# zxhuang1698/ShapeClipper

Measured on AMD Instinct MI355X. Metric: train-step images/sec (Pix3D cfg, bs32/GPU), higher is better.
Workload: dtype f32 (bf16x3-split MFMA, fp32 accumulate)

## Files before the change

### shapeclipper_amd/csrc/conv3x3_wgrad.hip

```cpp
#include <hip/hip_runtime.h>

#include "grid_cus.hpp"
#include "shapeclipper_hip.h"

namespace sc {

typedef float wg_f32x16 __attribute__((ext_vector_type(16)));

#ifdef SC_WGRAD_PROFILE
__device__ unsigned long long* wgrad_prof_buf = nullptr;
#define WG_STAMP(ID) { const unsigned long long t_ = __builtin_amdgcn_s_memrealtime(); if (wgrad_prof_buf && tid == 0) wgrad_prof_buf[(size_t)blockIdx.x * 16 + (ID)] = t_; }
#define WG_ACCUM(ID, T0) { const unsigned long long t_ = __builtin_amdgcn_s_memrealtime(); if (wgrad_prof_buf && tid == 0) wgrad_prof_buf[(size_t)blockIdx.x * 16 + (ID)] += t_ - (T0); }
#else
#define WG_STAMP(ID)
#endif

template <int W_, int NR_, int NIMG_, int GS_, int S_ = 1>
struct WgCfg {
    static constexpr int W = W_, H = W_, NR = NR_, NIMG = NIMG_, GS = GS_, S = S_;
    static constexpr int HW = W * W;
    static constexpr int XW = S * W, XH = S * H, XHW = XW * XH;
    static constexpr int Wp = S == 1 ? W + 2 : XW + 1;
    static constexpr bool WHOLE = NR == H;
    static constexpr int SLOTW = (W + 2 * GS - 1) / (2 * GS) * (2 * GS);
    static constexpr int ROWS = NIMG * NR;
    static constexpr int NSLOT = ROWS * SLOTW;
    static constexpr int GST = NSLOT + (((NSLOT / GS) & 1) ? 0 : GS);
    static constexpr int PR = S == 1 ? NR + 2 : 2 * NR + 1;
    static constexpr int PATCH = NIMG * PR * Wp;
    static constexpr int LQ = (S == 1 ? PATCH : PATCH + 2 * GS + 2) | 1;
    static constexpr int LDS_FLOATS = 64 * GST + 64 * LQ > 4 * 48 * 64 ? 64 * GST + 64 * LQ : 4 * 48 * 64;
    static constexpr int CHUNK = W == 7 ? 49 : 56;
    static constexpr int RPC = CHUNK / W;
    static constexpr int XCHUNK = XW == 7 ? 49 : 56, XRPC = XCHUNK / XW;
    static constexpr int XROWS = WHOLE ? XH : PR;
    static constexpr int XCH = (XROWS + XRPC - 1) / XRPC, GCH = (NR + RPC - 1) / RPC;
    static constexpr int HR = ROWS / 2;
    static constexpr int GPR = SLOTW / (2 * GS);
    static constexpr int KH_A = HR * SLOTW;
    static constexpr int KH_B = NIMG == 2 ? PR * Wp : S * HR * Wp;
    static constexpr int NBV = S == 1 ? GS + 2 : 2 * GS + 1;
    static_assert(ROWS % 2 == 0 && H % NR == 0 && SLOTW % (2 * GS) == 0 && CHUNK % W == 0 && XCHUNK % XW == 0 && (S == 1 || S == 2), "K-step shape");
    static_assert(LDS_FLOATS * 4 <= 160 * 1024 && 4 * 48 * 64 <= LDS_FLOATS, "LDS");
};

template <class C>
__global__ __launch_bounds__(512, 1) void conv3x3_wgrad_kernel(const float* __restrict__ gy, const float* __restrict__ x,
                                                               float* __restrict__ partial, int batch, int cin, int cout, int S) {
    constexpr int W = C::W, H = C::H, HW = C::HW, Wp = C::Wp, GS = C::GS, NIMG = C::NIMG, NR = C::NR, ST = C::S;
    constexpr int XW = C::XW, XH = C::XH, XHW = C::XHW;
    extern __shared__ float4 wg_smem[];
    float* As = reinterpret_cast<float*>(wg_smem);
    float* Xs = As + 64 * C::GST;
    const int tid = threadIdx.x, lane = tid & 63, wave = __builtin_amdgcn_readfirstlane(tid >> 6), half = lane >> 5;
    const int wt = wave & 3, kh = wave >> 2;
    const int nti = cin / 64;
    const int blk = blockIdx.x / S, s = blockIdx.x - blk * S;
    const int co0 = (blk / nti) * 64, ci0 = (blk % nti) * 64;
    const int nimg_steps = NIMG == 2 ? (batch + 1) / 2 : batch * (H / NR);
    const int k_lo = (int)((long long)s * nimg_steps / S), k_hi = (int)((long long)(s + 1) * nimg_steps / S);

    for (int i = tid; i < C::LDS_FLOATS; i += 512) As[i] = 0.f;

    const bool lane_on = lane < C::CHUNK, xlane_on = lane < C::XCHUNK;
    const int lrow = lane / W, lx = lane - lrow * W;
    const int xlrow = lane / XW, xlx = lane - xlrow * XW;
    float xv[8][C::XCH * NIMG], gv[8][C::GCH * NIMG];
    auto load = [&](int kstep) {
        int b, y0;
        if (NIMG == 2) { b = 2 * kstep; y0 = 0; } else { b = kstep / (H / NR); y0 = (kstep - b * (H / NR)) * NR; }
#pragma unroll
        for (int im = 0; im < NIMG; ++im) {
            const bool img_ok = b + im < batch;
            const float* xb = x + ((size_t)(b + im) * cin + ci0 + 8 * wave) * XHW;
            const float* gb = gy + ((size_t)(b + im) * cout + co0 + 8 * wave) * HW;
#pragma unroll
            for (int c = 0; c < C::XCH; ++c) {
                const int yr = (C::WHOLE ? 0 : ST * y0 - 1) + c * C::XRPC + xlrow;
                const bool ok = xlane_on && img_ok && (unsigned)yr < (unsigned)XH && c * C::XRPC + xlrow < C::XROWS;
                const int off = yr * XW + xlx;
#pragma unroll
                for (int ch = 0; ch < 8; ++ch) xv[ch][im * C::XCH + c] = ok ? xb[ch * XHW + off] : 0.f;
            }
#pragma unroll
            for (int c = 0; c < C::GCH; ++c) {
                const int yr = y0 + c * C::RPC + lrow;
                const bool ok = lane_on && img_ok && c * C::RPC + lrow < NR;
                const int off = yr * W + lx;
#pragma unroll
                for (int ch = 0; ch < 8; ++ch) gv[ch][im * C::GCH + c] = ok ? gb[ch * HW + off] : 0.f;
            }
        }
    };
    auto store = [&]() {
#pragma unroll
        for (int im = 0; im < NIMG; ++im) {
#pragma unroll
            for (int c = 0; c < C::XCH; ++c) {
                const int pr = (C::WHOLE ? 1 : 0) + c * C::XRPC + xlrow;
                if (xlane_on && c * C::XRPC + xlrow < C::XROWS) {
#pragma unroll
                    for (int ch = 0; ch < 8; ++ch) Xs[(8 * wave + ch) * C::LQ + (im * C::PR + pr) * Wp + 1 + xlx] = xv[ch][im * C::XCH + c];
                }
            }
#pragma unroll
            for (int c = 0; c < C::GCH; ++c) {
                if (lane_on && c * C::RPC + lrow < NR) {
#pragma unroll
                    for (int ch = 0; ch < 8; ++ch) As[(8 * wave + ch) * C::GST + (im * NR + c * C::RPC + lrow) * C::SLOTW + lx] = gv[ch][im * C::GCH + c];
                }
            }
        }
    };

    wg_f32x16 acc[9];
#pragma unroll
    for (int t = 0; t < 9; ++t)
#pragma unroll
        for (int r = 0; r < 16; ++r) acc[t][r] = 0.f;

    const float* Ab = As + ((wt >> 1) * 32 + (lane & 31)) * C::GST + half * GS + kh * C::KH_A;
    const float* Bb = Xs + ((wt & 1) * 32 + (lane & 31)) * C::LQ + half * ST * GS + kh * C::KH_B;

    if (k_lo < k_hi) load(k_lo);
    __syncthreads();
    for (int kstep = k_lo; kstep < k_hi; ++kstep) {
        store();
        __syncthreads();
        if (kstep + 1 < k_hi) load(kstep + 1);
#pragma unroll
        for (int yr = 0; yr < C::HR; ++yr) {
#pragma unroll
            for (int gx = 0; gx < C::GPR; ++gx) {
                float a[GS];
                if constexpr (GS == 4) {
                    const float4 t = *reinterpret_cast<const float4*>(Ab + yr * C::SLOTW + gx * 8);
                    a[0] = t.x, a[1] = t.y, a[2] = t.z, a[3] = t.w;
                } else if constexpr (GS == 2) {
                    const float2 t = *reinterpret_cast<const float2*>(Ab + yr * C::SLOTW + gx * 4);
                    a[0] = t.x, a[1] = t.y;
                } else {
                    a[0] = Ab[yr * C::SLOTW + gx * 2];
                }
#pragma unroll
                for (int ky = 0; ky < 3; ++ky) {
                    float bv[C::NBV];
#pragma unroll
                    for (int t = 0; t < C::NBV; ++t) bv[t] = Bb[(ST * yr + ky) * Wp + ST * gx * 2 * GS + t];
#pragma unroll
                    for (int ss = 0; ss < GS; ++ss)
#pragma unroll
                        for (int kx = 0; kx < 3; ++kx)
                            acc[ky * 3 + kx] = __builtin_amdgcn_mfma_f32_32x32x2f32(a[ss], bv[ST * ss + kx], acc[ky * 3 + kx], 0, 0, 0);
                }
            }
        }
        __syncthreads();
    }

    float* R = As;
#pragma unroll
    for (int pass = 0; pass < 3; ++pass) {
        if (kh == 1) {
#pragma unroll
            for (int t = 0; t < 3; ++t)
#pragma unroll
                for (int r = 0; r < 16; ++r) R[((wt * 3 + t) * 16 + r) * 64 + lane] = acc[pass * 3 + t][r];
        }
        __syncthreads();
        if (kh == 0) {
#pragma unroll
            for (int t = 0; t < 3; ++t)
#pragma unroll
                for (int r = 0; r < 16; ++r) acc[pass * 3 + t][r] += R[((wt * 3 + t) * 16 + r) * 64 + lane];
        }
        __syncthreads();
    }
    if (kh == 0) {
        float* dst = partial + (size_t)blockIdx.x * (64 * 64 * 9);
#pragma unroll
        for (int t = 0; t < 9; ++t)
#pragma unroll
            for (int r = 0; r < 16; ++r) dst[((wt * 9 + t) * 16 + r) * 64 + lane] = acc[t][r];
    }
}

__global__ __launch_bounds__(256) void conv3x3_wgrad_reduce_kernel(const float* __restrict__ partial, float* __restrict__ dw, int cin,
                                                                  int cout, int S) {
    __shared__ float part[4][64];
    const int nti = cin / 64, lane = threadIdx.x & 63, w = threadIdx.x >> 6;
    const int blk = blockIdx.x / 576, e = (blockIdx.x - blk * 576) * 64 + lane;
    const float* src = partial + (size_t)blk * S * 36864 + e;
    float s0 = 0.f, s1 = 0.f;
    int s = w;
    for (; s + 4 < S; s += 8) {
        s0 += src[(size_t)s * 36864];
        s1 += src[(size_t)(s + 4) * 36864];
    }
    if (s < S) s0 += src[(size_t)s * 36864];
    part[w][lane] = s0 + s1;
    __syncthreads();
    if (w == 0) {
        const float sum = (part[0][lane] + part[1][lane]) + (part[2][lane] + part[3][lane]);
        const int r = (e >> 6) & 15, t = (e >> 10) % 9, wt = e / (9 * 1024);
        const int co = (blk / nti) * 64 + (wt >> 1) * 32 + (r & 3) + 8 * (r >> 2) + 4 * (lane >> 5);
        const int ci = (blk % nti) * 64 + (wt & 1) * 32 + (lane & 31);
        dw[((size_t)co * cin + ci) * 9 + t] = sum;
    }
}

using Wg56 = WgCfg<56, 2, 1, 4>;
using Wg28 = WgCfg<28, 4, 1, 2>;
using Wg14 = WgCfg<14, 14, 1, 1>;
using Wg7 = WgCfg<7, 7, 2, 1>;
using Wg28S2 = WgCfg<28, 2, 1, 2, 2>;
using Wg14S2 = WgCfg<14, 2, 1, 1, 2>;
using Wg7S2 = WgCfg<7, 7, 2, 1, 2>;

typedef __bf16 wg_bf16x8 __attribute__((ext_vector_type(8)));
typedef float wg_f32x4 __attribute__((ext_vector_type(4)));
#ifndef SC_WGRAD_S16
#define SC_WGRAD_S16 0
#endif

template <int W_, int NR_, int NIMG_>
struct WsCfg {
    static constexpr int W = W_, H = W_, NR = NR_, NIMG = NIMG_, HW = W * W;
    static constexpr int SLOTS = W == 7 ? 8 : (W + 15) / 16 * 16;
    static constexpr int ROWS = NIMG * NR, NSLOT = ROWS * SLOTS, G = NSLOT / 16;
    static constexpr int ASTR = NSLOT + 8;
    static constexpr int Wp = SLOTS + 2, PR = NR + 2, PATCH = NIMG * PR * Wp;
    static constexpr int BSTR = (PATCH + 3) / 4 * 4 + 2;
    static constexpr bool WHOLE = NR == H;
    static constexpr int LDS_BYTES = 3 * 64 * (ASTR + BSTR) * 2;
    static constexpr int CHUNK = W == 7 ? 49 : 56, RPC = CHUNK / W;
    static constexpr int XROWS = WHOLE ? H : PR;
    static constexpr int XCH = (XROWS + RPC - 1) / RPC, GCH = (NR + RPC - 1) / RPC;
    static_assert(NSLOT % 16 == 0 && H % NR == 0 && LDS_BYTES <= 160 * 1024 && (W >= 14 || (NIMG == 2 && NR == 7)), "K-step shape");
    static constexpr int boff(int g, int h) {
        if (W == 7) { const int r = 2 * g + h; return ((r / 7) * PR + r % 7) * Wp; }
        const int r = g / (SLOTS / 16), gx = g % (SLOTS / 16);
        return ((r / NR) * PR + r % NR) * Wp + 16 * gx + 8 * h;
    }
};

template <class C>
__global__ __launch_bounds__(768, 1) void conv3x3_wgrad_split_kernel(const float* __restrict__ gy, const float* __restrict__ x,
                                                                     float* __restrict__ partial, int batch, int cin, int cout, int S) {
    constexpr int W = C::W, H = C::H, HW = C::HW, Wp = C::Wp, NIMG = C::NIMG, NR = C::NR;
    extern __shared__ float4 wg_smem[];
    __bf16* As = reinterpret_cast<__bf16*>(wg_smem);
    __bf16* Xs = As + 3 * 64 * C::ASTR;
    const int tid = threadIdx.x, lane = tid & 63, wave = __builtin_amdgcn_readfirstlane(tid >> 6), half = lane >> 5;
    const int wt = wave & 3, ky = wave >> 2;
    const int nti = cin / 64;
    const int blk = blockIdx.x / S, s = blockIdx.x - blk * S;
    const int co0 = (blk / nti) * 64, ci0 = (blk % nti) * 64;
    const int nimg_steps = NIMG == 2 ? (batch + 1) / 2 : batch * (H / NR);
    const int k_lo = (int)((long long)s * nimg_steps / S), k_hi = (int)((long long)(s + 1) * nimg_steps / S);

    for (int i = tid; i < C::LDS_BYTES / 16; i += 768) wg_smem[i] = make_float4(0.f, 0.f, 0.f, 0.f);

    const bool lane_on = lane < C::CHUNK, xrole = wave < 8;
    const int lrow = lane / W, lx = lane - lrow * W;
    constexpr int NSV = 8 * C::XCH * NIMG > 16 * C::GCH * NIMG ? 8 * C::XCH * NIMG : 16 * C::GCH * NIMG;
    float sv[NSV];
    auto load = [&](int kstep) {
        int b, y0;
        if (NIMG == 2) { b = 2 * kstep; y0 = 0; } else { b = kstep / (H / NR); y0 = (kstep - b * (H / NR)) * NR; }
        if (xrole) {
#pragma unroll
            for (int im = 0; im < NIMG; ++im) {
                const float* xb = x + ((size_t)(b + im) * cin + ci0 + 8 * wave) * HW;
#pragma unroll
                for (int c = 0; c < C::XCH; ++c) {
                    const int rr = c * C::RPC + lrow, yr = (C::WHOLE ? 0 : y0 - 1) + rr;
                    const bool ok = lane_on && b + im < batch && (unsigned)yr < (unsigned)H && rr < C::XROWS;
                    const int off = yr * W + lx;
#pragma unroll
                    for (int ch = 0; ch < 8; ++ch) sv[(im * C::XCH + c) * 8 + ch] = ok ? xb[ch * HW + off] : 0.f;
                }
            }
        } else {
#pragma unroll
            for (int im = 0; im < NIMG; ++im) {
                const float* gb = gy + ((size_t)(b + im) * cout + co0 + 16 * (wave - 8)) * HW;
#pragma unroll
                for (int c = 0; c < C::GCH; ++c) {
                    const int rr = c * C::RPC + lrow;
                    const bool ok = lane_on && b + im < batch && rr < NR;
                    const int off = (y0 + rr) * W + lx;
#pragma unroll
                    for (int ch = 0; ch < 16; ++ch) sv[(im * C::GCH + c) * 16 + ch] = ok ? gb[ch * HW + off] : 0.f;
                }
            }
        }
    };
    auto put = [&](__bf16* d, int stride, float v) {
        const __bf16 h0 = (__bf16)v;
        const float r1 = v - (float)h0;
        const __bf16 h1 = (__bf16)r1;
        d[0] = h0; d[stride] = h1; d[2 * stride] = (__bf16)(r1 - (float)h1);
    };
    auto store = [&]() {
        if (xrole) {
#pragma unroll
            for (int im = 0; im < NIMG; ++im)
#pragma unroll
                for (int c = 0; c < C::XCH; ++c) {
                    const int rr = c * C::RPC + lrow;
                    if (lane_on && rr < C::XROWS) {
                        __bf16* d = Xs + 8 * wave * C::BSTR + (im * C::PR + (C::WHOLE ? 1 : 0) + rr) * Wp + 1 + lx;
#pragma unroll
                        for (int ch = 0; ch < 8; ++ch) put(d + ch * C::BSTR, 64 * C::BSTR, sv[(im * C::XCH + c) * 8 + ch]);
                    }
                }
        } else {
#pragma unroll
            for (int im = 0; im < NIMG; ++im)
#pragma unroll
                for (int c = 0; c < C::GCH; ++c) {
                    const int rr = c * C::RPC + lrow;
                    if (lane_on && rr < NR) {
                        __bf16* d = As + 16 * (wave - 8) * C::ASTR + (im * NR + rr) * C::SLOTS + lx;
#pragma unroll
                        for (int ch = 0; ch < 16; ++ch) put(d + ch * C::ASTR, 64 * C::ASTR, sv[(im * C::GCH + c) * 16 + ch]);
                    }
                }
        }
    };

#if SC_WGRAD_S16
    wg_f32x4 acc[3][2][2];
#pragma unroll
    for (int t = 0; t < 3; ++t)
#pragma unroll
        for (int u = 0; u < 4; ++u) acc[t][u >> 1][u & 1] = wg_f32x4{0.f, 0.f, 0.f, 0.f};
    const int q4 = lane >> 4, l16 = lane & 15;
    const __bf16* Ab = As + ((wt >> 1) * 32 + l16) * C::ASTR + 8 * q4;
    const unsigned* Bb = reinterpret_cast<const unsigned*>(Xs + ((wt & 1) * 32 + l16) * C::BSTR + ky * Wp);
#else
    wg_f32x16 acc[3];
#pragma unroll
    for (int t = 0; t < 3; ++t)
#pragma unroll
        for (int r = 0; r < 16; ++r) acc[t][r] = 0.f;

    const __bf16* Ab = As + ((wt >> 1) * 32 + (lane & 31)) * C::ASTR + 8 * half;
    const unsigned* Bb = reinterpret_cast<const unsigned*>(Xs + ((wt & 1) * 32 + (lane & 31)) * C::BSTR + ky * Wp);
#endif

    WG_STAMP(0)
    if (k_lo < k_hi) load(k_lo);
    __syncthreads();
    WG_STAMP(1)
    for (int kstep = k_lo; kstep < k_hi; ++kstep) {
#ifdef SC_WGRAD_PROFILE
        const unsigned long long ts0 = __builtin_amdgcn_s_memrealtime();
#endif
        store();
        __syncthreads();
#ifdef SC_WGRAD_PROFILE
        WG_ACCUM(4, ts0)
        const unsigned long long ts1 = __builtin_amdgcn_s_memrealtime();
#endif
        if (kstep + 1 < k_hi) load(kstep + 1);
#if SC_WGRAD_S16
#pragma unroll
        for (int G2 = 0; G2 < (C::G + 1) / 2; ++G2) {
            constexpr int NG = C::G;
            const bool tail = 2 * G2 + 1 >= NG;
            const bool dead = tail && q4 >= 2;
            const int g1 = tail ? 2 * G2 : 2 * G2 + 1;
            const int bo = (q4 == 0 ? C::boff(2 * G2, 0) : q4 == 1 ? C::boff(2 * G2, 1) : q4 == 2 ? C::boff(g1, 0) : C::boff(g1, 1)) >> 1;
            float4 a[3][2];
#pragma unroll
            for (int pc = 0; pc < 3; ++pc)
#pragma unroll
                for (int u = 0; u < 2; ++u) {
                    const float4 av = *reinterpret_cast<const float4*>(Ab + pc * 64 * C::ASTR + u * 16 * C::ASTR + (dead ? 0 : 32 * G2));
                    a[pc][u] = dead ? make_float4(0.f, 0.f, 0.f, 0.f) : av;
                }
#pragma unroll
            for (int sb = 0; sb < 2; ++sb) {
                unsigned d[3][5];
#pragma unroll
                for (int pc = 0; pc < 3; ++pc)
#pragma unroll
                    for (int q = 0; q < 5; ++q) d[pc][q] = Bb[pc * 32 * C::BSTR + sb * 8 * C::BSTR + bo + q];
#pragma unroll
                for (int term = 0; term < 6; ++term) {
                    constexpr int PA[6] = {0, 2, 1, 0, 1, 0}, PB[6] = {2, 0, 1, 1, 0, 0};
                    const unsigned* q = d[PB[term]];
                    const uint4 b0 = {q[0], q[1], q[2], q[3]}, b2 = {q[1], q[2], q[3], q[4]};
                    const uint4 b1 = {__builtin_amdgcn_alignbit(q[1], q[0], 16), __builtin_amdgcn_alignbit(q[2], q[1], 16),
                                      __builtin_amdgcn_alignbit(q[3], q[2], 16), __builtin_amdgcn_alignbit(q[4], q[3], 16)};
#pragma unroll
                    for (int sa = 0; sa < 2; ++sa) {
                        const wg_bf16x8 av = __builtin_bit_cast(wg_bf16x8, a[PA[term]][sa]);
                        acc[0][sa][sb] = __builtin_amdgcn_mfma_f32_16x16x32_bf16(av, __builtin_bit_cast(wg_bf16x8, b0), acc[0][sa][sb], 0, 0, 0);
                        acc[1][sa][sb] = __builtin_amdgcn_mfma_f32_16x16x32_bf16(av, __builtin_bit_cast(wg_bf16x8, b1), acc[1][sa][sb], 0, 0, 0);
                        acc[2][sa][sb] = __builtin_amdgcn_mfma_f32_16x16x32_bf16(av, __builtin_bit_cast(wg_bf16x8, b2), acc[2][sa][sb], 0, 0, 0);
                    }
                }
#pragma unroll
                for (int pc = 0; pc < 3; ++pc)
                    asm volatile("" : "+v"(acc[0][0][sb]) : "v"(d[pc][0]), "v"(d[pc][1]), "v"(d[pc][2]), "v"(d[pc][3]), "v"(d[pc][4]));
            }
#pragma unroll
            for (int pc = 0; pc < 3; ++pc)
                asm volatile("" : "+v"(acc[0][0][0]) : "v"(__builtin_bit_cast(wg_f32x4, a[pc][0])), "v"(__builtin_bit_cast(wg_f32x4, a[pc][1])));
            __builtin_amdgcn_sched_barrier(0);
        }
#else
#pragma unroll
        for (int g = 0; g < C::G; ++g) {
            float4 a[3];
            unsigned d[3][5];
            const int bo = (half ? C::boff(g, 1) : C::boff(g, 0)) >> 1;
#pragma unroll
            for (int pc = 0; pc < 3; ++pc) {
                a[pc] = *reinterpret_cast<const float4*>(Ab + pc * 64 * C::ASTR + 16 * g);
#pragma unroll
                for (int q = 0; q < 5; ++q) d[pc][q] = Bb[pc * 32 * C::BSTR + bo + q];
            }
#pragma unroll
            for (int term = 0; term < 6; ++term) {
                constexpr int PA[6] = {0, 2, 1, 0, 1, 0}, PB[6] = {2, 0, 1, 1, 0, 0};
                const unsigned* q = d[PB[term]];
                const wg_bf16x8 av = __builtin_bit_cast(wg_bf16x8, a[PA[term]]);
                uint4 b0 = {q[0], q[1], q[2], q[3]}, b2 = {q[1], q[2], q[3], q[4]};
                uint4 b1 = {__builtin_amdgcn_alignbit(q[1], q[0], 16), __builtin_amdgcn_alignbit(q[2], q[1], 16),
                            __builtin_amdgcn_alignbit(q[3], q[2], 16), __builtin_amdgcn_alignbit(q[4], q[3], 16)};
                acc[0] = __builtin_amdgcn_mfma_f32_32x32x16_bf16(av, __builtin_bit_cast(wg_bf16x8, b0), acc[0], 0, 0, 0);
                acc[1] = __builtin_amdgcn_mfma_f32_32x32x16_bf16(av, __builtin_bit_cast(wg_bf16x8, b1), acc[1], 0, 0, 0);
                acc[2] = __builtin_amdgcn_mfma_f32_32x32x16_bf16(av, __builtin_bit_cast(wg_bf16x8, b2), acc[2], 0, 0, 0);
            }
        }
#endif
        __syncthreads();
#ifdef SC_WGRAD_PROFILE
        WG_ACCUM(5, ts1)
#endif
    }
    WG_STAMP(2)
    float* dst = partial + (size_t)blockIdx.x * (64 * 64 * 9);
#if SC_WGRAD_S16
#pragma unroll
    for (int t = 0; t < 3; ++t)
#pragma unroll
        for (int sa = 0; sa < 2; ++sa)
#pragma unroll
            for (int sb = 0; sb < 2; ++sb)
#pragma unroll
                for (int r = 0; r < 4; ++r)
                    dst[((wt * 9 + ky * 3 + t) * 16 + r + 4 * (2 * sa + (q4 >> 1))) * 64 + 16 * sb + l16 + 32 * (q4 & 1)] = acc[t][sa][sb][r];
#else
#pragma unroll
    for (int t = 0; t < 3; ++t)
#pragma unroll
        for (int r = 0; r < 16; ++r) dst[((wt * 9 + ky * 3 + t) * 16 + r) * 64 + lane] = acc[t][r];
#endif
#ifdef SC_WGRAD_PROFILE
    asm volatile("s_waitcnt vmcnt(0)" ::: "memory");
    WG_STAMP(3)
    if (wgrad_prof_buf && tid == 0) wgrad_prof_buf[(size_t)blockIdx.x * 16 + 6] = (unsigned long long)(k_hi - k_lo);
#endif
}

using Ws56 = WsCfg<56, 2, 1>;
using Ws28 = WsCfg<28, 4, 1>;
using Ws14 = WsCfg<14, 7, 1>;
using Ws7 = WsCfg<7, 7, 2>;

static int wg_cus() { return grid_cus(); }
static int wg_splits(int cin, int cout) {
    const int nblk = (cin / 64) * (cout / 64), s = wg_cus() / nblk;
    return s > 0 ? s : 1;
}

template <class C>
static int launch_wgrad(const float* gy, const float* x, float* dw, float* workspace, int batch, int cin, int cout, hipStream_t st) {
    if (cin % 64 || cout % 64 || batch <= 0) return (int)hipErrorInvalidValue;
    const int nblk = (cin / 64) * (cout / 64), S = wg_splits(cin, cout);
    (void)hipFuncSetAttribute((const void*)conv3x3_wgrad_kernel<C>, hipFuncAttributeMaxDynamicSharedMemorySize, C::LDS_FLOATS * 4);
    hipLaunchKernelGGL((conv3x3_wgrad_kernel<C>), dim3(nblk * S), dim3(512), C::LDS_FLOATS * 4, st, gy, x, workspace, batch, cin, cout, S);
    hipLaunchKernelGGL(conv3x3_wgrad_reduce_kernel, dim3(nblk * 576), dim3(256), 0, st, workspace, dw, cin, cout, S);
    return (int)hipGetLastError();
}

template <class C>
static int launch_wgrad_split(const float* gy, const float* x, float* dw, float* workspace, int batch, int cin, int cout, hipStream_t st) {
    if (cin % 64 || cout % 64 || batch <= 0) return (int)hipErrorInvalidValue;
    const int nblk = (cin / 64) * (cout / 64), S = wg_splits(cin, cout);
    (void)hipFuncSetAttribute((const void*)conv3x3_wgrad_split_kernel<C>, hipFuncAttributeMaxDynamicSharedMemorySize, C::LDS_BYTES);
    hipLaunchKernelGGL((conv3x3_wgrad_split_kernel<C>), dim3(nblk * S), dim3(768), C::LDS_BYTES, st, gy, x, workspace, batch, cin, cout, S);
    hipLaunchKernelGGL(conv3x3_wgrad_reduce_kernel, dim3(nblk * 576), dim3(256), 0, st, workspace, dw, cin, cout, S);
    return (int)hipGetLastError();
}

}

#ifdef SC_WGRAD_PROFILE
extern "C" int sc_wgrad_debug_set_prof(unsigned long long* buf) {
    return (int)hipMemcpyToSymbol(HIP_SYMBOL(sc::wgrad_prof_buf), &buf, sizeof(buf));
}
#endif
extern "C" int sc_conv3x3_wgrad_split(const float* gy, const float* x, float* dw, float* workspace, int batch, int cin, int cout, int hw, void* stream) {
    switch (hw) {
        case 56: return sc::launch_wgrad_split<sc::Ws56>(gy, x, dw, workspace, batch, cin, cout, (hipStream_t)stream);
        case 28: return sc::launch_wgrad_split<sc::Ws28>(gy, x, dw, workspace, batch, cin, cout, (hipStream_t)stream);
        case 14: return sc::launch_wgrad_split<sc::Ws14>(gy, x, dw, workspace, batch, cin, cout, (hipStream_t)stream);
        case 7: return sc::launch_wgrad_split<sc::Ws7>(gy, x, dw, workspace, batch, cin, cout, (hipStream_t)stream);
        default: return -1;
    }
}

extern "C" long long sc_conv3x3_wgrad_workspace_floats(int cin, int cout) {
    if (cin <= 0 || cout <= 0 || cin % 64 || cout % 64) return -1;
    return (long long)(cin / 64) * (cout / 64) * sc::wg_splits(cin, cout) * 36864;
}

extern "C" int sc_conv3x3s2_wgrad(const float* gy, const float* x, float* dw, float* workspace, int batch, int cin, int cout, int hw, void* stream) {
    switch (hw) {
        case 56: return sc::launch_wgrad<sc::Wg28S2>(gy, x, dw, workspace, batch, cin, cout, (hipStream_t)stream);
        case 28: return sc::launch_wgrad<sc::Wg14S2>(gy, x, dw, workspace, batch, cin, cout, (hipStream_t)stream);
        case 14: return sc::launch_wgrad<sc::Wg7S2>(gy, x, dw, workspace, batch, cin, cout, (hipStream_t)stream);
        default: return -1;
    }
}

extern "C" int sc_conv3x3_wgrad(const float* gy, const float* x, float* dw, float* workspace, int batch, int cin, int cout, int hw, void* stream) {
    switch (hw) {
        case 56: return sc::launch_wgrad<sc::Wg56>(gy, x, dw, workspace, batch, cin, cout, (hipStream_t)stream);
        case 28: return sc::launch_wgrad<sc::Wg28>(gy, x, dw, workspace, batch, cin, cout, (hipStream_t)stream);
        case 14: return sc::launch_wgrad<sc::Wg14>(gy, x, dw, workspace, batch, cin, cout, (hipStream_t)stream);
        case 7: return sc::launch_wgrad<sc::Wg7>(gy, x, dw, workspace, batch, cin, cout, (hipStream_t)stream);
        default: return -1;
    }
}
```

Baseline: 1037.

## Deal wgrad staging loads across waves in channel pairs and precompute B-operand addresses

Adds a paired load and store path for the split wgrad kernel, used by the 28 and 14 configs. Each wave now loads contiguous pixel runs for pairs of channels, with both wave classes sharing the x and gy work, and splits two values at once into bf16x3 using packed converts and 32-bit LDS stores. It also removes the unused 16x16 MFMA variant and reworks the B-operand fetch to two 4-word loads from precomputed byte offsets, deriving the shifted operand by alignbit. This is meant to cut global-load imbalance, per-element split cost and LDS address arithmetic, at the price of more template parameters and higher register pressure in the staging buffer.

```diff
diff --git a/shapeclipper_amd/csrc/conv3x3_wgrad.hip b/shapeclipper_amd/csrc/conv3x3_wgrad.hip
--- a/shapeclipper_amd/csrc/conv3x3_wgrad.hip
+++ b/shapeclipper_amd/csrc/conv3x3_wgrad.hip
@@ -218,12 +218,10 @@
 using Wg7S2 = WgCfg<7, 7, 2, 1, 2>;
 
 typedef __bf16 wg_bf16x8 __attribute__((ext_vector_type(8)));
-typedef float wg_f32x4 __attribute__((ext_vector_type(4)));
-#ifndef SC_WGRAD_S16
-#define SC_WGRAD_S16 0
-#endif
-
-template <int W_, int NR_, int NIMG_>
+typedef __bf16 wg_bf16x2 __attribute__((ext_vector_type(2)));
+typedef float wg_f32x2 __attribute__((ext_vector_type(2)));
+template <int N> struct wg_int { static constexpr int value = N; };
+template <int W_, int NR_, int NIMG_, int XPA_, int XPB_, int GA_, int GB_, bool PAIRED_, bool TW_>
 struct WsCfg {
     static constexpr int W = W_, H = W_, NR = NR_, NIMG = NIMG_, HW = W * W;
     static constexpr int SLOTS = W == 7 ? 8 : (W + 15) / 16 * 16;
@@ -233,10 +231,25 @@
     static constexpr int BSTR = (PATCH + 3) / 4 * 4 + 2;
     static constexpr bool WHOLE = NR == H;
     static constexpr int LDS_BYTES = 3 * 64 * (ASTR + BSTR) * 2;
+    static constexpr int XROWS = WHOLE ? H : PR;
+    static constexpr int XL = XROWS * W, GL = NR * W;
+    static constexpr bool GPIX = W % 2 == 0;
+    static constexpr int GPL = GPIX ? 2 : 1;
+    static constexpr int XCW = XL % 56 == 0 && XL / 56 == (XL + 63) / 64 ? 56 : 64;
+    static constexpr int XCH = (XL + XCW - 1) / XCW, GCH = (GL + 64 * GPL - 1) / (64 * GPL);
+    static constexpr int XU = XCH * NIMG, GU = GCH * NIMG;
+    static constexpr int XPA = XPA_, XPB = XPB_, GA = GA_, GB = GB_;
+    static constexpr bool PAIRED = PAIRED_;
+    static constexpr bool TW = TW_;
+    static constexpr int XPM = XPA > XPB ? XPA : XPB, GM = GA > GB ? GA : GB;
+    static constexpr int NSVP = 2 * (GM * GU + XPM * XU);
     static constexpr int CHUNK = W == 7 ? 49 : 56, RPC = CHUNK / W;
-    static constexpr int XROWS = WHOLE ? H : PR;
-    static constexpr int XCH = (XROWS + RPC - 1) / RPC, GCH = (NR + RPC - 1) / RPC;
+    static constexpr int RXCH = (XROWS + RPC - 1) / RPC, RGCH = (NR + RPC - 1) / RPC;
+    static constexpr int NSVR = 8 * RXCH * NIMG > 16 * RGCH * NIMG ? 8 * RXCH * NIMG : 16 * RGCH * NIMG;
+    static constexpr int NSV = PAIRED ? NSVP : NSVR;
+    static constexpr int HD = W == 7 ? Wp / 2 : 4;
     static_assert(NSLOT % 16 == 0 && H % NR == 0 && LDS_BYTES <= 160 * 1024 && (W >= 14 || (NIMG == 2 && NR == 7)), "K-step shape");
+    static_assert(8 * XPA + 4 * XPB == 32 && 8 * GA + 4 * GB == (GPIX ? 64 : 32) && (!GPIX || (GL % 2 == 0 && SLOTS % 2 == 0 && ASTR % 2 == 0)), "dealing");
     static constexpr int boff(int g, int h) {
         if (W == 7) { const int r = 2 * g + h; return ((r / 7) * PR + r % 7) * Wp; }
         const int r = g / (SLOTS / 16), gx = g % (SLOTS / 16);
@@ -261,24 +274,128 @@
 
     for (int i = tid; i < C::LDS_BYTES / 16; i += 768) wg_smem[i] = make_float4(0.f, 0.f, 0.f, 0.f);
 
-    const bool lane_on = lane < C::CHUNK, xrole = wave < 8;
-    const int lrow = lane / W, lx = lane - lrow * W;
-    constexpr int NSV = 8 * C::XCH * NIMG > 16 * C::GCH * NIMG ? 8 * C::XCH * NIMG : 16 * C::GCH * NIMG;
-    float sv[NSV];
-    auto load = [&](int kstep) {
+    static_assert(C::GCH == 1, "a gy unit is one chunk per image");
+    const bool cls_a = wave < 8;
+    const int xp0 = cls_a ? wave * C::XPA : 8 * C::XPA + (wave - 8) * C::XPB;
+    const int gu0 = cls_a ? wave * C::GA : 8 * C::GA + (wave - 8) * C::GB;
+    int xrr[C::XCH], xlo[C::XCH];
+#pragma unroll
+    for (int c = 0; c < C::XCH; ++c) {
+        if constexpr (C::XCW % W == 0) {
+            xrr[c] = c * (C::XCW / W) + (C::XCW == W ? 0 : lane / W);
+            xlo[c] = ((C::WHOLE ? 1 : 0) + c * (C::XCW / W)) * Wp + (C::XCW == W ? 0 : lane / W * Wp) + 1 + (C::XCW == W ? lane : lane % W);
+        } else {
+            const int e = C::XCW * c + lane;
+            xrr[c] = e / W;
+            xlo[c] = ((C::WHOLE ? 1 : 0) + xrr[c]) * Wp + 1 + e - xrr[c] * W;
+        }
+    }
+    auto x_on = [&](int c) { return (C::XCW == 64 || lane < C::XCW) && (C::XCW * c + C::XCW - 1 < C::XL || lane < C::XL - C::XCW * c); };
+    const int ge = C::GPL * lane, grr = ge / W, glo = grr * C::SLOTS + ge - grr * W;
+    const bool g_on = ge < C::GL;
+    float sv[C::NSV];
+    auto load_as = [&](auto nxp, auto ng, int kstep) {
+        constexpr int NXP = decltype(nxp)::value, NG = decltype(ng)::value, XPM = C::XPM, GM = C::GM, X0 = 2 * GM * C::GU;
         int b, y0;
         if (NIMG == 2) { b = 2 * kstep; y0 = 0; } else { b = kstep / (H / NR); y0 = (kstep - b * (H / NR)) * NR; }
-        if (xrole) {
+#pragma unroll
+        for (int im = 0; im < NIMG; ++im) {
+            const bool img_ok = b + im < batch;
+            if constexpr (NXP > 0) {
+                const float* xb = x + ((size_t)(b + im) * cin + ci0 + 2 * xp0) * HW + (C::WHOLE ? 0 : (y0 - 1) * W) + lane;
+#pragma unroll
+                for (int c = 0; c < C::XCH; ++c) {
+                    const bool ok = x_on(c) && img_ok && (C::WHOLE || (unsigned)(y0 - 1 + xrr[c]) < (unsigned)H);
+#pragma unroll
+                    for (int q = 0; q < 2 * NXP; ++q) sv[X0 + (im * C::XCH + c) * XPM * 2 + q] = ok ? xb[q * HW + C::XCW * c] : 0.f;
+                }
+            }
+            if constexpr (NG > 0) {
+                const bool ok = g_on && img_ok;
+                if constexpr (C::GPIX) {
+                    const float* gb = gy + ((size_t)(b + im) * cout + co0 + gu0) * HW + y0 * W + 2 * lane;
+#pragma unroll
+                    for (int u = 0; u < NG; ++u) {
+                        const wg_f32x2 t = ok ? *reinterpret_cast<const wg_f32x2*>(gb + u * HW) : wg_f32x2{0.f, 0.f};
+                        sv[(im * GM + u) * 2] = t.x, sv[(im * GM + u) * 2 + 1] = t.y;
+                    }
+                } else {
+                    const float* gb = gy + ((size_t)(b + im) * cout + co0 + 2 * gu0) * HW + y0 * W + lane;
+#pragma unroll
+                    for (int q = 0; q < 2 * NG; ++q) sv[im * GM * 2 + q] = ok ? gb[q * HW] : 0.f;
+                }
+            }
+        }
+        asm volatile("");
+    };
+    auto split2 = [&](float v0, float v1, unsigned (&h)[3]) {
+        wg_f32x2 v = {v0, v1};
+#pragma unroll
+        for (int pc = 0; pc < 3; ++pc) {
+            h[pc] = __builtin_bit_cast(unsigned, __builtin_convertvector(v, wg_bf16x2));
+            if (pc < 2) v = v - wg_f32x2{__builtin_bit_cast(float, h[pc] << 16), __builtin_bit_cast(float, h[pc] & 0xffff0000u)};
+        }
+    };
+    auto store_as = [&](auto nxp, auto ng) {
+        constexpr int NXP = decltype(nxp)::value, NG = decltype(ng)::value, XPM = C::XPM, GM = C::GM, X0 = 2 * GM * C::GU;
+        unsigned short* xs16 = reinterpret_cast<unsigned short*>(Xs) + 2 * xp0 * C::BSTR;
+        unsigned short* as16 = reinterpret_cast<unsigned short*>(As) + (C::GPIX ? 1 : 2) * gu0 * C::ASTR;
+#pragma unroll
+        for (int im = 0; im < NIMG; ++im) {
+            if constexpr (NXP > 0) {
+#pragma unroll
+                for (int c = 0; c < C::XCH; ++c)
+                    if (x_on(c)) {
+                        unsigned short* d = xs16 + im * C::PR * Wp + xlo[c];
+#pragma unroll
+                        for (int p = 0; p < NXP; ++p) {
+                            unsigned h[3];
+                            split2(sv[X0 + ((im * C::XCH + c) * XPM + p) * 2], sv[X0 + ((im * C::XCH + c) * XPM + p) * 2 + 1], h);
+#pragma unroll
+                            for (int pc = 0; pc < 3; ++pc) {
+                                d[(pc * 64 + 2 * p) * C::BSTR] = (unsigned short)h[pc];
+                                d[(pc * 64 + 2 * p + 1) * C::BSTR] = (unsigned short)(h[pc] >> 16);
+                            }
+                        }
+                    }
+            }
+            if constexpr (NG > 0) {
+                if (g_on) {
+                    unsigned short* d = as16 + im * NR * C::SLOTS + glo;
+#pragma unroll
+                    for (int u = 0; u < NG; ++u) {
+                        unsigned h[3];
+                        split2(sv[(im * GM + u) * 2], sv[(im * GM + u) * 2 + 1], h);
+#pragma unroll
+                        for (int pc = 0; pc < 3; ++pc) {
+                            if constexpr (C::GPIX) {
+                                *reinterpret_cast<unsigned*>(d + (pc * 64 + u) * C::ASTR) = h[pc];
+                            } else {
+                                d[(pc * 64 + 2 * u) * C::ASTR] = (unsigned short)h[pc];
+                                d[(pc * 64 + 2 * u + 1) * C::ASTR] = (unsigned short)(h[pc] >> 16);
+                            }
+                        }
+                    }
+                }
+            }
+        }
+    };
+    const bool lane_on = lane < C::CHUNK;
+    const int lrow = lane / W, lx = lane - lrow * W;
+    auto load_rows = [&](int kstep) {
+        int b, y0;
+        if (NIMG == 2) { b = 2 * kstep; y0 = 0; } else { b = kstep / (H / NR); y0 = (kstep - b * (H / NR)) * NR; }
+        if (cls_a) {
 #pragma unroll
             for (int im = 0; im < NIMG; ++im) {
                 const float* xb = x + ((size_t)(b + im) * cin + ci0 + 8 * wave) * HW;
 #pragma unroll
-                for (int c = 0; c < C::XCH; ++c) {
+                for (int c = 0; c < C::RXCH; ++c) {
                     const int rr = c * C::RPC + lrow, yr = (C::WHOLE ? 0 : y0 - 1) + rr;
                     const bool ok = lane_on && b + im < batch && (unsigned)yr < (unsigned)H && rr < C::XROWS;
                     const int off = yr * W + lx;
 #pragma unroll
-                    for (int ch = 0; ch < 8; ++ch) sv[(im * C::XCH + c) * 8 + ch] = ok ? xb[ch * HW + off] : 0.f;
+                    for (int ch = 0; ch < 8; ++ch) sv[(im * C::RXCH + c) * 8 + ch] = ok ? xb[ch * HW + off] : 0.f;
                 }
             }
         } else {
@@ -286,12 +403,12 @@
             for (int im = 0; im < NIMG; ++im) {
                 const float* gb = gy + ((size_t)(b + im) * cout + co0 + 16 * (wave - 8)) * HW;
 #pragma unroll
-                for (int c = 0; c < C::GCH; ++c) {
+                for (int c = 0; c < C::RGCH; ++c) {
                     const int rr = c * C::RPC + lrow;
                     const bool ok = lane_on && b + im < batch && rr < NR;
                     const int off = (y0 + rr) * W + lx;
 #pragma unroll
-                    for (int ch = 0; ch < 16; ++ch) sv[(im * C::GCH + c) * 16 + ch] = ok ? gb[ch * HW + off] : 0.f;
+                    for (int ch = 0; ch < 16; ++ch) sv[(im * C::RGCH + c) * 16 + ch] = ok ? gb[ch * HW + off] : 0.f;
                 }
             }
         }
@@ -302,53 +419,58 @@
         const __bf16 h1 = (__bf16)r1;
         d[0] = h0; d[stride] = h1; d[2 * stride] = (__bf16)(r1 - (float)h1);
     };
-    auto store = [&]() {
-        if (xrole) {
+    auto store_rows = [&]() {
+        if (cls_a) {
 #pragma unroll
             for (int im = 0; im < NIMG; ++im)
 #pragma unroll
-                for (int c = 0; c < C::XCH; ++c) {
+                for (int c = 0; c < C::RXCH; ++c) {
                     const int rr = c * C::RPC + lrow;
                     if (lane_on && rr < C::XROWS) {
                         __bf16* d = Xs + 8 * wave * C::BSTR + (im * C::PR + (C::WHOLE ? 1 : 0) + rr) * Wp + 1 + lx;
 #pragma unroll
-                        for (int ch = 0; ch < 8; ++ch) put(d + ch * C::BSTR, 64 * C::BSTR, sv[(im * C::XCH + c) * 8 + ch]);
+                        for (int ch = 0; ch < 8; ++ch) put(d + ch * C::BSTR, 64 * C::BSTR, sv[(im * C::RXCH + c) * 8 + ch]);
                     }
                 }
         } else {
 #pragma unroll
             for (int im = 0; im < NIMG; ++im)
 #pragma unroll
-                for (int c = 0; c < C::GCH; ++c) {
+                for (int c = 0; c < C::RGCH; ++c) {
                     const int rr = c * C::RPC + lrow;
                     if (lane_on && rr < NR) {
                         __bf16* d = As + 16 * (wave - 8) * C::ASTR + (im * NR + rr) * C::SLOTS + lx;
 #pragma unroll
-                        for (int ch = 0; ch < 16; ++ch) put(d + ch * C::ASTR, 64 * C::ASTR, sv[(im * C::GCH + c) * 16 + ch]);
+                        for (int ch = 0; ch < 16; ++ch) put(d + ch * C::ASTR, 64 * C::ASTR, sv[(im * C::RGCH + c) * 16 + ch]);
                     }
                 }
         }
     };
-
-#if SC_WGRAD_S16
-    wg_f32x4 acc[3][2][2];
+    auto load = [&](int kstep) {
+        if constexpr (!C::PAIRED) load_rows(kstep);
+        else if (cls_a) load_as(wg_int<C::XPA>{}, wg_int<C::GA>{}, kstep); else load_as(wg_int<C::XPB>{}, wg_int<C::GB>{}, kstep);
+    };
+    auto store = [&]() {
+        if constexpr (!C::PAIRED) store_rows();
+        else if (cls_a) store_as(wg_int<C::XPA>{}, wg_int<C::GA>{}); else store_as(wg_int<C::XPB>{}, wg_int<C::GB>{});
+    };
+
+    wg_f32x16 acc[3];
 #pragma unroll
     for (int t = 0; t < 3; ++t)
 #pragma unroll
-        for (int u = 0; u < 4; ++u) acc[t][u >> 1][u & 1] = wg_f32x4{0.f, 0.f, 0.f, 0.f};
-    const int q4 = lane >> 4, l16 = lane & 15;
-    const __bf16* Ab = As + ((wt >> 1) * 32 + l16) * C::ASTR + 8 * q4;
-    const unsigned* Bb = reinterpret_cast<const unsigned*>(Xs + ((wt & 1) * 32 + l16) * C::BSTR + ky * Wp);
-#else
-    wg_f32x16 acc[3];
-#pragma unroll
-    for (int t = 0; t < 3; ++t)
-#pragma unroll
         for (int r = 0; r < 16; ++r) acc[t][r] = 0.f;
 
     const __bf16* Ab = As + ((wt >> 1) * 32 + (lane & 31)) * C::ASTR + 8 * half;
+    const char* smem_b = reinterpret_cast<const char*>(wg_smem);
     const unsigned* Bb = reinterpret_cast<const unsigned*>(Xs + ((wt & 1) * 32 + (lane & 31)) * C::BSTR + ky * Wp);
-#endif
+    int xq[3], xq2[3];
+#pragma unroll
+    for (int pc = 0; pc < 3 && C::TW; ++pc) {
+        xq[pc] = 2 * (3 * 64 * C::ASTR + (pc * 64 + (wt & 1) * 32 + (lane & 31)) * C::BSTR + ky * Wp) + 4 * C::HD * half;
+        xq2[pc] = xq[pc] + 4;
+        asm volatile("" : "+v"(xq[pc]), "+v"(xq2[pc]));
+    }
 
     WG_STAMP(0)
     if (k_lo < k_hi) load(k_lo);
@@ -365,79 +487,39 @@
         const unsigned long long ts1 = __builtin_amdgcn_s_memrealtime();
 #endif
         if (kstep + 1 < k_hi) load(kstep + 1);
-#if SC_WGRAD_S16
-#pragma unroll
-        for (int G2 = 0; G2 < (C::G + 1) / 2; ++G2) {
-            constexpr int NG = C::G;
-            const bool tail = 2 * G2 + 1 >= NG;
-            const bool dead = tail && q4 >= 2;
-            const int g1 = tail ? 2 * G2 : 2 * G2 + 1;
-            const int bo = (q4 == 0 ? C::boff(2 * G2, 0) : q4 == 1 ? C::boff(2 * G2, 1) : q4 == 2 ? C::boff(g1, 0) : C::boff(g1, 1)) >> 1;
-            float4 a[3][2];
-#pragma unroll
-            for (int pc = 0; pc < 3; ++pc)
-#pragma unroll
-                for (int u = 0; u < 2; ++u) {
-                    const float4 av = *reinterpret_cast<const float4*>(Ab + pc * 64 * C::ASTR + u * 16 * C::ASTR + (dead ? 0 : 32 * G2));
-                    a[pc][u] = dead ? make_float4(0.f, 0.f, 0.f, 0.f) : av;
-                }
-#pragma unroll
-            for (int sb = 0; sb < 2; ++sb) {
-                unsigned d[3][5];
-#pragma unroll
-                for (int pc = 0; pc < 3; ++pc)
-#pragma unroll
-                    for (int q = 0; q < 5; ++q) d[pc][q] = Bb[pc * 32 * C::BSTR + sb * 8 * C::BSTR + bo + q];
-#pragma unroll
-                for (int term = 0; term < 6; ++term) {
-                    constexpr int PA[6] = {0, 2, 1, 0, 1, 0}, PB[6] = {2, 0, 1, 1, 0, 0};
-                    const unsigned* q = d[PB[term]];
-                    const uint4 b0 = {q[0], q[1], q[2], q[3]}, b2 = {q[1], q[2], q[3], q[4]};
-                    const uint4 b1 = {__builtin_amdgcn_alignbit(q[1], q[0], 16), __builtin_amdgcn_alignbit(q[2], q[1], 16),
-                                      __builtin_amdgcn_alignbit(q[3], q[2], 16), __builtin_amdgcn_alignbit(q[4], q[3], 16)};
-#pragma unroll
-                    for (int sa = 0; sa < 2; ++sa) {
-                        const wg_bf16x8 av = __builtin_bit_cast(wg_bf16x8, a[PA[term]][sa]);
-                        acc[0][sa][sb] = __builtin_amdgcn_mfma_f32_16x16x32_bf16(av, __builtin_bit_cast(wg_bf16x8, b0), acc[0][sa][sb], 0, 0, 0);
-                        acc[1][sa][sb] = __builtin_amdgcn_mfma_f32_16x16x32_bf16(av, __builtin_bit_cast(wg_bf16x8, b1), acc[1][sa][sb], 0, 0, 0);
-                        acc[2][sa][sb] = __builtin_amdgcn_mfma_f32_16x16x32_bf16(av, __builtin_bit_cast(wg_bf16x8, b2), acc[2][sa][sb], 0, 0, 0);
-                    }
-                }
-#pragma unroll
-                for (int pc = 0; pc < 3; ++pc)
-                    asm volatile("" : "+v"(acc[0][0][sb]) : "v"(d[pc][0]), "v"(d[pc][1]), "v"(d[pc][2]), "v"(d[pc][3]), "v"(d[pc][4]));
-            }
-#pragma unroll
-            for (int pc = 0; pc < 3; ++pc)
-                asm volatile("" : "+v"(acc[0][0][0]) : "v"(__builtin_bit_cast(wg_f32x4, a[pc][0])), "v"(__builtin_bit_cast(wg_f32x4, a[pc][1])));
-            __builtin_amdgcn_sched_barrier(0);
-        }
-#else
 #pragma unroll
         for (int g = 0; g < C::G; ++g) {
             float4 a[3];
-            unsigned d[3][5];
-            const int bo = (half ? C::boff(g, 1) : C::boff(g, 0)) >> 1;
+            uint4 w0[3], w2[3];
+            const int bo = C::boff(g, 0) >> 1;
+            const int bh = (C::boff(g, 1) >> 1)     - bo - C::HD;
+            const int bx = bh ? (half ? 4 * bh : 0) : 0;
 #pragma unroll
             for (int pc = 0; pc < 3; ++pc) {
                 a[pc] = *reinterpret_cast<const float4*>(Ab + pc * 64 * C::ASTR + 16 * g);
-#pragma unroll
-                for (int q = 0; q < 5; ++q) d[pc][q] = Bb[pc * 32 * C::BSTR + bo + q];
+                if constexpr (C::TW) {
+                    const unsigned* p0 = reinterpret_cast<const unsigned*>(smem_b + xq[pc] + bx) + bo;
+                    const unsigned* p2 = reinterpret_cast<const unsigned*>(smem_b + xq2[pc] + bx) + bo;
+                    w0[pc] = uint4{p0[0], p0[1], p0[2], p0[3]};
+                    w2[pc] = uint4{p2[0], p2[1], p2[2], p2[3]};
+                } else {
+                    const unsigned* p0 = Bb + pc * 32 * C::BSTR + (half ? C::boff(g, 1) : C::boff(g, 0)) / 2;
+                    w0[pc] = uint4{p0[0], p0[1], p0[2], p0[3]};
+                    w2[pc] = uint4{p0[1], p0[2], p0[3], p0[4]};
+                }
             }
 #pragma unroll
             for (int term = 0; term < 6; ++term) {
                 constexpr int PA[6] = {0, 2, 1, 0, 1, 0}, PB[6] = {2, 0, 1, 1, 0, 0};
-                const unsigned* q = d[PB[term]];
+                const uint4 b0 = w0[PB[term]], b2 = w2[PB[term]];
                 const wg_bf16x8 av = __builtin_bit_cast(wg_bf16x8, a[PA[term]]);
-                uint4 b0 = {q[0], q[1], q[2], q[3]}, b2 = {q[1], q[2], q[3], q[4]};
-                uint4 b1 = {__builtin_amdgcn_alignbit(q[1], q[0], 16), __builtin_amdgcn_alignbit(q[2], q[1], 16),
-                            __builtin_amdgcn_alignbit(q[3], q[2], 16), __builtin_amdgcn_alignbit(q[4], q[3], 16)};
+                const uint4 b1 = {__builtin_amdgcn_alignbit(b2.x, b0.x, 16), __builtin_amdgcn_alignbit(b2.y, b0.y, 16),
+                                  __builtin_amdgcn_alignbit(b2.z, b0.z, 16), __builtin_amdgcn_alignbit(b2.w, b0.w, 16)};
                 acc[0] = __builtin_amdgcn_mfma_f32_32x32x16_bf16(av, __builtin_bit_cast(wg_bf16x8, b0), acc[0], 0, 0, 0);
                 acc[1] = __builtin_amdgcn_mfma_f32_32x32x16_bf16(av, __builtin_bit_cast(wg_bf16x8, b1), acc[1], 0, 0, 0);
                 acc[2] = __builtin_amdgcn_mfma_f32_32x32x16_bf16(av, __builtin_bit_cast(wg_bf16x8, b2), acc[2], 0, 0, 0);
             }
         }
-#endif
         __syncthreads();
 #ifdef SC_WGRAD_PROFILE
         WG_ACCUM(5, ts1)
@@ -445,22 +527,10 @@
     }
     WG_STAMP(2)
     float* dst = partial + (size_t)blockIdx.x * (64 * 64 * 9);
-#if SC_WGRAD_S16
 #pragma unroll
     for (int t = 0; t < 3; ++t)
 #pragma unroll
-        for (int sa = 0; sa < 2; ++sa)
-#pragma unroll
-            for (int sb = 0; sb < 2; ++sb)
-#pragma unroll
-                for (int r = 0; r < 4; ++r)
-                    dst[((wt * 9 + ky * 3 + t) * 16 + r + 4 * (2 * sa + (q4 >> 1))) * 64 + 16 * sb + l16 + 32 * (q4 & 1)] = acc[t][sa][sb][r];
-#else
-#pragma unroll
-    for (int t = 0; t < 3; ++t)
-#pragma unroll
         for (int r = 0; r < 16; ++r) dst[((wt * 9 + ky * 3 + t) * 16 + r) * 64 + lane] = acc[t][r];
-#endif
 #ifdef SC_WGRAD_PROFILE
     asm volatile("s_waitcnt vmcnt(0)" ::: "memory");
     WG_STAMP(3)
@@ -468,10 +538,10 @@
 #endif
 }
 
-using Ws56 = WsCfg<56, 2, 1>;
-using Ws28 = WsCfg<28, 4, 1>;
-using Ws14 = WsCfg<14, 7, 1>;
-using Ws7 = WsCfg<7, 7, 2>;
+using Ws56 = WsCfg<56, 2, 1, 4, 0, 0, 16, false, false>;
+using Ws28 = WsCfg<28, 4, 1, 3, 2, 5, 6, true, true>;
+using Ws14 = WsCfg<14, 7, 1, 3, 2, 5, 6, true, true>;
+using Ws7 = WsCfg<7, 7, 2, 4, 0, 1, 6, false, false>;
 
 static int wg_cus() { return grid_cus(); }
 static int wg_splits(int cin, int cout) {
```

Result: slower. 1026 (-1.1%).
